# jgrss/cultionet

Hardware: AMD Instinct MI355X
Metric: train_chips_per_sec (higher is better)
Workload: dtype f32

## Files before the change

cultionet_amd/csrc/cn_conv.hip:

```cpp
#include "cn_common.h"
#include "cn_conv_geom.h"
#include "cn_profile.h"

#include <cstdlib>

#define KC 8

static int cn_reduce_slices(const CnConvGeom& g, hipStream_t stream);

template <int TN, int TM>
__device__ __forceinline__ void cn_igemm_epilogue(const CnConvGeom& g, const f32x16 (&acc)[TN][TM],
                                                  const bool (&pix_ok)[TM], const int (&out_off)[TM], int co_base,
                                                  int half, int grp, int split, int b,
                                                  const float* __restrict__ bias, float* __restrict__ y) {
  const int HWout = g.Hout * g.Wout;
  const bool sliced = g.slice_stride != 0;
  float* yb = sliced ? g.part + (long)(grp * g.splits + split) * g.slice_stride + (long)b * g.Cout * HWout
                     : y + (long)b * g.ybs;
  const bool first = split == 0;
#pragma unroll
  for (int tn = 0; tn < TN; ++tn) {
#pragma unroll
    for (int r = 0; r < 16; ++r) {
      const int co = co_base + tn * 32 + (r & 3) + 8 * (r >> 2) + 4 * half;
      if (co < g.Cout) {
        const float bv = (bias != nullptr && first) ? bias[co] : 0.f;
#pragma unroll
        for (int tm = 0; tm < TM; ++tm) {
          if (pix_ok[tm]) {
            float* dst = yb + (long)co * HWout + out_off[tm];
            const float v = acc[tn][tm][r] + bv;
            if (sliced) {
              *dst = acc[tn][tm][r];
            } else if (g.atomic_out) {
              atomicAdd(dst, v);
            } else if (g.accumulate) {
              *dst += v;
            } else {
              *dst = v;
            }
          }
        }
      }
    }
  }
}

template <int WAVES_N, int TN, int NI_T>
__global__ __launch_bounds__(256) void cn_conv_igemm_kernel(const CnConvGeom g) {
  constexpr int WAVES_M = 4 / WAVES_N;
  constexpr int MT = WAVES_M * 64;
  constexpr int NT = WAVES_N * TN * 32;
  constexpr int WI = (CN_MAX_TAPS * KC * (NT / 4) + 255) / 256;
  extern __shared__ __attribute__((aligned(16))) float smem[];
  float* in_lds = smem;
  float* w_lds = smem + g.w_lds_off;
  int* tap_lds = reinterpret_cast<int*>(smem + g.tap_lds_off);

  const int tid = threadIdx.x, lane = tid & 63, wid = tid >> 6;
// ... 131 lines not shown
  {                                                                                                        \
    const float* wrow = w_lds + ((t_) * KC + half) * NT + wn * (TN * 32) + l31;                            \
    _Pragma("unroll") for (int tn = 0; tn < TN; ++tn) opa[bf_][tn] = wrow[(2 * (cp_)) * NT + tn * 32];     \
    opb[bf_][0] = in_lds[pix_lds[0] + (2 * (cp_)) * plane + (toff_)];                                      \
    opb[bf_][1] = in_lds[pix_lds[1] + (2 * (cp_)) * plane + (toff_)];                                      \
  }
#define CN_MFMA(bf_)                                                                                       \
  _Pragma("unroll") for (int tn = 0; tn < TN; ++tn) _Pragma("unroll") for (int tm = 0; tm < 2; ++tm)       \
      acc[tn][tm] = __builtin_amdgcn_mfma_f32_32x32x2f32(opa[bf_][tn], opb[bf_][tm], acc[tn][tm], 0, 0, 0);
      int toff_cur = tap_lds[0];
      CN_LOAD_OPS(0, 0, 0, toff_cur);
#pragma unroll 1
      for (int t = 0; t < ntaps; ++t) {
        const int toff_nxt = (t + 1 < ntaps) ? tap_lds[t + 1] : 0;
        CN_LOAD_OPS(1, t, 1, toff_cur);
        CN_MFMA(0);
        CN_LOAD_OPS(0, t, 2, toff_cur);
        CN_MFMA(1);
        CN_LOAD_OPS(1, t, 3, toff_cur);
        CN_MFMA(0);
        if (t + 1 < ntaps) CN_LOAD_OPS(0, t + 1, 0, toff_nxt);
        CN_MFMA(1);
        toff_cur = toff_nxt;
      }
#undef CN_LOAD_OPS
#undef CN_MFMA
    }
#undef CN_PREFETCH
  }

  cn_igemm_epilogue<TN, 2>(g, acc, pix_ok, out_off, n0 + wn * (TN * 32), half, grp, split, b, bias, y);
}

template <int WAVES_N, int TN, int TM, int NV, int RP>
__global__ __launch_bounds__(256, (NV <= 1 ? 2 : 1)) void cn_conv_igemm_vec_kernel(const CnConvGeom g) {
  constexpr int WAVES_M = 4 / WAVES_N;
  constexpr int MT = WAVES_M * TM * 32;
  constexpr int NT = WAVES_N * TN * 32;
  constexpr int WI = (CN_MAX_TAPS * KC * (NT / 4) + 255) / 256;
  constexpr int VS = NV * 1024;
  constexpr bool PADR = RP == 1 || RP == 2;
  constexpr int ODD = RP == 3 ? 1 : 0;
  constexpr int VSS = VS + ODD;
  extern __shared__ __attribute__((aligned(16))) float smem[];
  float* in_lds = smem;
  float* w_lds = smem + g.w_lds_off;
  int* tap_lds = reinterpret_cast<int*>(smem + g.tap_lds_off);

  const int tid = threadIdx.x, lane = tid & 63, wid = tid >> 6;
  const int half = lane >> 5, l31 = lane & 31;
  const int wm = wid / WAVES_N, wn = wid % WAVES_N;

  int bx, by, split;
  if (!cn_xcd_block(g.grid_x, g.grid_y, g.grid_x * g.grid_y * g.splits, bx, by, split)) return;
  int ci_ = 0;
  if (g.interleave) {
    ci_ = bx % g.ncls;
  } else {
#pragma unroll 1
    for (int c = 1; c < g.ncls; ++c)
      if (bx >= g.cls[c].block_begin) ci_ = c;
  }
  const int grp = g.cls[ci_].grp;
  const float* __restrict__ x = g.gx[grp];
  const float* __restrict__ wp = g.gwp[grp];
  const float* __restrict__ bias = g.gbias[grp];
  float* __restrict__ y = g.gy[grp];
  const int Hg = g.cls[ci_].Hg, Wg = g.cls[ci_].Wg, ntaps = g.cls[ci_].ntaps;
  const int vplane = g.cls[ci_].vplane;
  const int min_dy = g.cls[ci_].min_dy, min_dx = g.cls[ci_].min_dx;
  const int oy0 = g.cls[ci_].oy0, ox0 = g.cls[ci_].ox0;
  const int tiles_per_img = g.cls[ci_].tiles_per_img;
  const int tile = g.interleave ? bx / g.ncls : bx - g.cls[ci_].block_begin;
  const int b = tile / tiles_per_img;
  const int m0 = (tile - b * tiles_per_img) * MT;
  const int Win = g.Win;
  const int pitch = PADR ? ((Win + 3) / 4 * 4 + 4) : Win;
  if (tid < ntaps) {
    tap_lds[tid] = PADR ? (g.cls[ci_].dy[tid] - min_dy) * pitch + g.cls[ci_].dx[tid]
                      : (g.cls[ci_].dy[tid] - min_dy) * Win + (g.cls[ci_].dx[tid] - min_dx);
    tap_lds[CN_MAX_TAPS + tid] = g.cls[ci_].wt[tid];
    tap_lds[2 * CN_MAX_TAPS + tid] = g.cls[ci_].dx[tid];
  }
  __syncthreads();
  const int n0 = by * NT;
  const int Mimg = Hg * Wg;
  const int gy0 = m0 / Wg;
  const int HWin = g.Hin * Win;
  const int start = PADR ? (gy0 * g.is + min_dy) * Win : (gy0 * g.is + min_dy) * Win + min_dx;
  const int f0 = (start >> 2) << 2;
  const int sh = start - f0;

  int goff[NV];
  int ldst[NV];
  int ldst2[NV];
#pragma unroll
  for (int i = 0; i < NV; ++i) {
    const int e4 = 4 * (tid + i * 256) - (PADR ? sh : 0);
    const int lim = PADR ? g.cls[ci_].rows * Win : vplane;
    ldst[i] = 0;
    ldst2[i] = 0;
    if (e4 + 3 >= 0 && e4 < lim) {
      const int fq = start + e4 - (PADR ? 0 : sh);
      goff[i] = (fq >= 0 && (ODD ? fq < HWin : fq + 3 < HWin)) ? fq : -1;
      if (RP == 1) {
        const int r = e4 / Win;
        ldst[i] = r * pitch + 4 + (e4 - r * Win);
      } else if (RP == 2) {
        const int ea = e4 < 0 ? e4 + 2 : e4, eb = e4 + 2;
        const int ra = ea / Win, rb = eb / Win;
        ldst[i] = e4 < 0 ? -1 : ra * pitch + 4 + (ea - ra * Win);
        ldst2[i] = eb < lim ? rb * pitch + 4 + (eb - rb * Win) : -1;
      } else {
        ldst[i] = e4;
      }
    } else {
      goff[i] = -2;
    }
  }
  if (PADR) {
    for (int e = tid; e < KC * VS; e += 256) in_lds[e] = 0.f;
  }

  int pix_lds[TM], out_off[TM];
  unsigned colmask[TM];
  bool pix_ok[TM];
#pragma unroll
  for (int tm = 0; tm < TM; ++tm) {
    const int p = m0 + wm * (TM * 32) + tm * 32 + l31;
    pix_ok[tm] = p < Mimg;
    const int pc = pix_ok[tm] ? p : Mimg - 1;
    const int gy = pc / Wg, gx = pc - gy * Wg;
    pix_lds[tm] = PADR ? ((gy - gy0) * g.is) * pitch + 4 + gx * g.is + half * VS
                     : ((gy - gy0) * g.is) * Win + gx * g.is + sh + half * VSS;
    out_off[tm] = (gy * g.os + oy0) * g.Wout + gx * g.os + ox0;
    unsigned m = 0;
    for (int t = 0; t < ntaps; ++t) {
      const int ix = gx * g.is + tap_lds[2 * CN_MAX_TAPS + t];
      if (ix >= 0 && ix < Win) m |= 1u << t;
    }
    colmask[tm] = m;
  }

  f32x16 acc[TN][TM];
#pragma unroll
  for (int tn = 0; tn < TN; ++tn)
#pragma unroll
    for (int tm = 0; tm < TM; ++tm)
#pragma unroll
      for (int r = 0; r < 16; ++r) acc[tn][tm][r] = 0.f;
  const float* xb = x + (long)b * g.xbs;
  const int nw4 = ntaps * KC * (NT / 4);
  const int nchunks = (g.Cin + KC - 1) / KC;
  int ch = split * g.chunks_per_split;
  int ch_end = ch + g.chunks_per_split;
  if (ch_end > nchunks) ch_end = nchunks;

  if (ntaps > 0 && ch < ch_end) {
    f32x4 xin[KC][NV];
    f32x4 win[WI];
    constexpr unsigned CN_OOB = 0x80000000u;
    const __amdgpu_buffer_rsrc_t xrs =
        __builtin_amdgcn_make_buffer_rsrc(const_cast<float*>(xb), 0, 0x7fffffff, 0x00020000);
    const __amdgpu_buffer_rsrc_t wrs =
        __builtin_amdgcn_make_buffer_rsrc(const_cast<float*>(wp), 0, 0x7fffffff, 0x00020000);
    unsigned xo[NV], wo[WI];
#pragma unroll
    for (int i = 0; i < NV; ++i) xo[i] = goff[i] >= 0 ? (unsigned)goff[i] * 4u : CN_OOB;
#pragma unroll
    for (int j = 0; j < WI; ++j) {
      const int f = tid + j * 256;
      wo[j] = CN_OOB;
      if (f < nw4) {
        const int row = f / (NT / 4), c4 = f - row * (NT / 4);
        const int t = row / KC, ci = row - t * KC;
        wo[j] = (unsigned)(((tap_lds[CN_MAX_TAPS + t] * g.Kpad + ci) * g.Npad + n0 + c4 * 4) * 4);
      }
    }
#define CN_PREFETCH_V(c0_)                                                                                 \
  {                                                                                                        \
    const int c0 = (c0_);                                                                                  \
    _Pragma("unroll") for (int ci = 0; ci < KC; ++ci) {                                                    \
      if ((c0 + ci) < g.Cin) {                                                           \
        const int so = ODD ? (((c0 + ci) * HWin) & ~3) * 4 : (c0 + ci) * HWin * 4;                                                               \
        _Pragma("unroll") for (int i = 0; i < NV; ++i)                                                     \
            xin[ci][i] = __builtin_bit_cast(f32x4, __builtin_amdgcn_raw_buffer_load_b128(xrs, xo[i], so, 0)); \
      } else {                                                                                             \
        _Pragma("unroll") for (int i = 0; i < NV; ++i) xin[ci][i] = f32x4{0.f, 0.f, 0.f, 0.f};             \
      }                                                                                                    \
    }                                                                                                      \
    const int wso = c0 * g.Npad * 4;                                                                       \
    _Pragma("unroll") for (int j = 0; j < WI; ++j)                                                         \
        win[j] = __builtin_bit_cast(f32x4, __builtin_amdgcn_raw_buffer_load_b128(wrs, wo[j], wso, 0));     \
  }
    CN_PREFETCH_V(ch * KC);
    for (; ch < ch_end; ++ch) {
      __syncthreads();
#pragma unroll
      for (int ci = 0; ci < KC; ++ci)
#pragma unroll
        for (int i = 0; i < NV; ++i)
          if (goff[i] != -2) {
            if (RP == 2) {
              if (ldst[i] >= 0) *reinterpret_cast<float2*>(in_lds + ci * VS + ldst[i]) = make_float2(xin[ci][i][0], xin[ci][i][1]);
// ... 17 lines not shown
        if (f < nw4) *reinterpret_cast<f32x4*>(w_lds + f * 4) = win[j];
      }
      __syncthreads();
      if (ch + 1 < ch_end) CN_PREFETCH_V((ch + 1) * KC);
#pragma unroll 1
      for (int t = 0; t < ntaps; ++t) {
        const int toff = tap_lds[t];
        const float* wrow = w_lds + (t * KC + half) * NT + wn * (TN * 32) + l31;
        const float* brow[TM];
        int msk[TM];
#pragma unroll
        for (int tm = 0; tm < TM; ++tm) {
          brow[tm] = in_lds + pix_lds[tm] + toff;
          msk[tm] = PADR ? -1 : __builtin_amdgcn_sbfe((int)colmask[tm], t, 1);
        }
#pragma unroll
        for (int cp = 0; cp < KC / 2; ++cp) {
          float a[TN], bb[TM];
#pragma unroll
          for (int tn = 0; tn < TN; ++tn) a[tn] = wrow[(2 * cp) * NT + tn * 32];
#pragma unroll
          for (int tm = 0; tm < TM; ++tm)
            bb[tm] = PADR ? brow[tm][(2 * cp) * VS] : __int_as_float(__float_as_int(brow[tm][(2 * cp) * VSS]) & msk[tm]);
#pragma unroll
          for (int tn = 0; tn < TN; ++tn)
#pragma unroll
            for (int tm = 0; tm < TM; ++tm)
              acc[tn][tm] = __builtin_amdgcn_mfma_f32_32x32x2f32(a[tn], bb[tm], acc[tn][tm], 0, 0, 0);
        }
      }
    }
#undef CN_PREFETCH_V
  }

  cn_igemm_epilogue<TN, TM>(g, acc, pix_ok, out_off, n0 + wn * (TN * 32), half, grp, split, b, bias, y);
}

__global__ void cn_pack_weights_kernel(const float* __restrict__ w, float* __restrict__ wp, int T, int K,
                                       int N, int Kpad, int Npad, long sk, long sn, long st) {
  const long total = (long)T * Kpad * Npad;
  for (long i = blockIdx.x * (long)blockDim.x + threadIdx.x; i < total; i += (long)gridDim.x * blockDim.x) {
    const int n = (int)(i % Npad);
    const long r = i / Npad;
    const int k = (int)(r % Kpad);
    const int t = (int)(r / Kpad);
    wp[i] = (k < K && n < N) ? w[k * sk + n * sn + t * st] : 0.f;
  }
}

struct CnPackDesc {
  const float* w;
  float* wp;
  int T, K, N, Kpad, Npad;
  long sk, sn, st;
};

#define CN_PK_TS 32
#define CN_PK_PITCH (32 * CN_MAX_TAPS + 1)
__global__ __launch_bounds__(256) void cn_pack_weights_batched_kernel(const CnPackDesc* __restrict__ descs) {
  __shared__ float tile[CN_PK_TS * CN_PK_PITCH];
  const CnPackDesc d = descs[blockIdx.y];
  const bool n_slow = d.sn > d.sk;
  const long ss = n_slow ? d.sn : d.sk, sm = n_slow ? d.sk : d.sn;
  const int S = n_slow ? d.N : d.K, M = n_slow ? d.K : d.N;
  const int Spad = n_slow ? d.Npad : d.Kpad, Mpad = n_slow ? d.Kpad : d.Npad;
  if (d.T > CN_MAX_TAPS || d.st != 1 || sm != d.T) {
    const long total = (long)d.T * d.Kpad * d.Npad;
    for (long i = blockIdx.x * (long)blockDim.x + threadIdx.x; i < total; i += (long)gridDim.x * blockDim.x) {
// ... 33 lines not shown

extern "C" int cn_conv_npad(int n_out) {
  const int nt = cn_pick_nt(n_out);
  return (n_out + nt - 1) / nt * nt;
}
extern "C" int cn_conv_kpad(int k_in) { return (k_in + KC - 1) / KC * KC; }

extern "C" int cn_pack_weights_f32(const float* w, float* wp, int T, int K, int N, long sk, long sn, long st,
                                   void* stream) {
  const int Kpad = cn_conv_kpad(K), Npad = cn_conv_npad(N);
  const long total = (long)T * Kpad * Npad;
  const int blocks = (int)((total + 255) / 256 < 2048 ? (total + 255) / 256 : 2048);
  CN_LAUNCH(cn_pack_weights_kernel, dim3(blocks), dim3(256), 0, (hipStream_t)stream, w, wp, T, K, N,
                     Kpad, Npad, sk, sn, st);
  return cn_check_launch();
}

extern "C" int cn_pack_weights_batched_f32(const void* descs, int n, void* stream) {
  if (n <= 0) return CN_OK;
  CN_LAUNCH(cn_pack_weights_batched_kernel, dim3(64, n), dim3(256), 0, (hipStream_t)stream,
                     (const CnPackDesc*)descs);
  return cn_check_launch();
}

template <int WAVES_N, int TN, int TM, int NV, int RP>
static int cn_launch_igemm_v(const float* x, const float* wp, const float* bias, float* y, CnConvGeom& g,
                             int total_tiles, int max_taps, int splits, double flops, hipStream_t stream) {
  constexpr int NT = WAVES_N * TN * 32;
  g.tap_lds_off = g.w_lds_off + (max_taps > 0 ? max_taps : 1) * KC * NT;
  if ((long)g.Cin * g.Hin * g.Win * 4 >= (1L << 31) || (long)(max_taps > 0 ? max_taps : 1) * g.Kpad * g.Npad * 4 >= (1L << 31))
    return CN_ERR_ARG;
  const size_t lds = (size_t)(g.tap_lds_off + 3 * CN_MAX_TAPS + 1) * sizeof(float);
  if (lds > 160 * 1024) return CN_ERR_LDS;
  static bool attr_set = false;
  if (!attr_set) {
    (void)hipFuncSetAttribute((const void*)cn_conv_igemm_vec_kernel<WAVES_N, TN, TM, NV, RP>,
                              hipFuncAttributeMaxDynamicSharedMemorySize, 160 * 1024);
    attr_set = true;
  }
  g.grid_x = total_tiles;
  g.grid_y = (g.Cout + NT - 1) / NT;
  g.splits = splits < 1 ? 1 : splits;
  dim3 grid(cn_xcd_grid((long)g.grid_x * g.grid_y * g.splits));
  cn_prof_name("cn_conv_igemm_vec_kernel<%d, %d, %d, %d, %d>", WAVES_N, TN, TM, NV, RP);
  cn_prof_desc("igemm_vec<%d,%d,%d,%d,%d> G%d B%d %d->%d %dx%d->%dx%d taps%d cls%d is%d os%d grid%dx%dx%d", WAVES_N, TN,
               TM, NV, RP, g.G, g.B, g.Cin, g.Cout, g.Hin, g.Win, g.Hout, g.Wout, max_taps, g.ncls, g.is, g.os,
               total_tiles, (g.Cout + NT - 1) / NT, splits);
  cn_prof_bytes(4.0 * g.G * ((double)g.B * g.Cin * g.Hin * g.Win + (double)g.B * g.Cout * g.Hout * g.Wout / (g.shared_y ? g.G : 1) +
                             (double)(max_taps > 0 ? max_taps : 1) * g.Cin * g.Cout));
  cn_prof_before(stream);
  CN_LAUNCH((cn_conv_igemm_vec_kernel<WAVES_N, TN, TM, NV, RP>), grid, dim3(256), lds, stream, g);
  cn_prof_after(stream, NT == 128 ? 0 : 1, flops);
  const int rrc = cn_reduce_slices(g, stream);
  return rrc != CN_OK ? rrc : cn_check_launch();
}

template <int WAVES_N, int TN, int NI_T>
static int cn_launch_igemm_t(const float* x, const float* wp, const float* bias, float* y, CnConvGeom& g,
                             int total_tiles, int max_taps, int splits, double flops, hipStream_t stream) {
  constexpr int NT = WAVES_N * TN * 32;
  g.tap_lds_off = g.w_lds_off + (max_taps > 0 ? max_taps : 1) * KC * NT;
  if ((long)g.Cin * g.Hin * g.Win * 4 >= (1L << 31) || (long)(max_taps > 0 ? max_taps : 1) * g.Kpad * g.Npad * 4 >= (1L << 31))
    return CN_ERR_ARG;
  const size_t lds = (size_t)(g.tap_lds_off + 3 * CN_MAX_TAPS + 1) * sizeof(float);
  if (lds > 160 * 1024) return CN_ERR_LDS;
  static bool attr_set = false;
  if (!attr_set) {
    (void)hipFuncSetAttribute((const void*)cn_conv_igemm_kernel<WAVES_N, TN, NI_T>,
                              hipFuncAttributeMaxDynamicSharedMemorySize, 160 * 1024);
    attr_set = true;
  }
  g.grid_x = total_tiles;
  g.grid_y = (g.Cout + NT - 1) / NT;
  g.splits = splits < 1 ? 1 : splits;
  dim3 grid(cn_xcd_grid((long)g.grid_x * g.grid_y * g.splits));
  cn_prof_name("cn_conv_igemm_kernel<%d, %d, %d>", WAVES_N, TN, NI_T);
  cn_prof_desc("igemm_dw<%d,%d,%d> G%d B%d %d->%d %dx%d->%dx%d taps%d cls%d is%d os%d grid%dx%dx%d", WAVES_N, TN, NI_T,
               g.G, g.B, g.Cin, g.Cout, g.Hin, g.Win, g.Hout, g.Wout, max_taps, g.ncls, g.is, g.os, total_tiles,
               (g.Cout + NT - 1) / NT, splits);
  cn_prof_bytes(4.0 * g.G * ((double)g.B * g.Cin * g.Hin * g.Win + (double)g.B * g.Cout * g.Hout * g.Wout / (g.shared_y ? g.G : 1) +
                             (double)(max_taps > 0 ? max_taps : 1) * g.Cin * g.Cout));
  cn_prof_before(stream);
  CN_LAUNCH((cn_conv_igemm_kernel<WAVES_N, TN, NI_T>), grid, dim3(256), lds, stream, g);
  cn_prof_after(stream, NT == 128 ? 0 : 1, flops);
// ... 4 lines not shown
struct CnPlan {
  int total_tiles, max_plane, max_vplane, max_taps;
  int max_rplane, max_absdx;
  double flops;
};

static CnPlan cn_plan(CnConvGeom& g, int MT) {
  CnPlan p = {0, 0, 0, 0, 0, 0, 0.0};
  for (int c = 0; c < g.ncls; ++c) {
    CnConvClass& k = g.cls[c];
    const int Mimg = k.Hg * k.Wg;
    int rows_g = (MT + k.Wg - 2) / k.Wg + 1;
    if (rows_g > k.Hg) rows_g = k.Hg;
    k.min_dy = 0; k.min_dx = 0;
    int max_dy = 0, max_dx = 0;
    for (int t = 0; t < k.ntaps; ++t) {
      if (t == 0 || k.dy[t] < k.min_dy) k.min_dy = k.dy[t];
      if (t == 0 || k.dx[t] < k.min_dx) k.min_dx = k.dx[t];
      if (t == 0 || k.dy[t] > max_dy) max_dy = k.dy[t];
      if (t == 0 || k.dx[t] > max_dx) max_dx = k.dx[t];
    }
    const int rows = (rows_g - 1) * g.is + (max_dy - k.min_dy) + 1;
    k.pitch = (k.Wg - 1) * g.is + (max_dx - k.min_dx) + 1;
    k.plane = rows * k.pitch;
    k.vplane = (rows * g.Win + (max_dx - k.min_dx) + 4 + 3) / 4 * 4;
    k.rows = rows;
    {
      const int rpitch = (g.Win + 3) / 4 * 4 + 4;
      if ((rows + 1) * rpitch + 4 > p.max_rplane) p.max_rplane = (rows + 1) * rpitch + 4;
    }
    if (-k.min_dx > p.max_absdx) p.max_absdx = -k.min_dx;
    if (max_dx > p.max_absdx) p.max_absdx = max_dx;
    k.tiles_per_img = (Mimg + MT - 1) / MT;
    k.block_begin = p.total_tiles;
    p.total_tiles += g.B * k.tiles_per_img;
    if (k.plane > p.max_plane) p.max_plane = k.plane;
    if (k.vplane > p.max_vplane) p.max_vplane = k.vplane;
    if (k.ntaps > p.max_taps) p.max_taps = k.ntaps;
    p.flops += 2.0 * g.B * Mimg * (double)g.Cout * g.Cin * k.ntaps;
  }
  g.interleave = 0;
  if (g.ncls > 1 && g.want_interleave) {
    bool same = true;
    for (int c = 1; c < g.ncls; ++c) same = same && g.cls[c].tiles_per_img == g.cls[0].tiles_per_img;
    g.interleave = same ? 1 : 0;
  }
  return p;
}

struct CnChoice { int cfg, splits, cps; double cost; };

static double cn_launch_cost(long blocks, int cps, double mt_units, int splits, double out_elems) {
  const double F = 273.0, R = 170.0;
  const double c1 = 36.7 + 0.614 * mt_units, c2 = 30.0 + 1.19 * mt_units;
  const long full = blocks / 512, rem = blocks % 512;
  double c = full * (F + cps * c2);
  if (rem > 0) c += F + cps * (rem > 256 ? c2 : c1);
  if (splits > 1) c += R + out_elems * 4.0 * (2.0 * splits + 1.0) / 8.0e6 * (128.0 / 7.5);
  return c;
}

static thread_local float* g_conv_ws;
static thread_local long g_conv_ws_floats;

static CnChoice cn_choose(const CnConvGeom& g0, const int* mts, int ncfg, int NT, bool allow_split) {
  const int nchunks = (g0.Cin + KC - 1) / KC;
  const int ny = (g0.Cout + NT - 1) / NT;
  const int G = g0.G > 0 ? g0.G : 1;
  const double out_elems = (double)g0.B * g0.Cout * g0.Hout * g0.Wout * (g0.shared_y ? 1 : G);
  CnChoice best = {0, 1, nchunks > 0 ? nchunks : 1, 1e300};
  int forced = 0;
  {
    static const char* dbg = getenv("CN_DBG_SPLITS");
    if (dbg) forced = atoi(dbg) < 1 ? 1 : atoi(dbg);
  }
  long ws_cap = 32;
  if (g_conv_ws != nullptr) {
    const long stride = ((long)g0.B * g0.Cout * g0.Hout * g0.Wout + 3) / 4 * 4;
    ws_cap = g_conv_ws_floats / (stride * G);
  }
  int forced_cfg = -1;
  {
    static const char* dbgc = getenv("CN_DBG_CFG");
    if (dbgc) forced_cfg = atoi(dbgc);
  }
  for (int i = 0; i < ncfg; ++i) {
    if (forced_cfg >= 0 && i != (forced_cfg < ncfg ? forced_cfg : ncfg - 1)) continue;
    CnConvGeom gi = g0;
    const CnPlan p = cn_plan(gi, mts[i]);
    if (p.total_tiles <= 0) continue;
    const long base = (long)p.total_tiles * ny;
    int max_splits = (allow_split && p.max_taps > 0 && nchunks >= 4) ? nchunks / 2 : 1;
    if (max_splits > 32) max_splits = 32;
    if (max_splits > ws_cap) max_splits = ws_cap < 1 ? 1 : (int)ws_cap;
    const double taps = p.total_tiles > 0 ? p.flops / (2.0 * g0.Cout * g0.Cin * (double)mts[i] * p.total_tiles) : 9.0;
    const double chunk_units = (double)mts[i] * NT / 128.0 * (taps < 9.0 ? taps : 9.0) / 9.0;
    for (int sp = 1; sp <= max_splits; ++sp) {
      if (forced && sp != (forced > max_splits ? max_splits : forced)) continue;
      const int cps = (nchunks + sp - 1) / sp;
      const int splits = (nchunks + cps - 1) / cps;
      if (splits != sp && !forced) continue;
      const double cost = cn_launch_cost(base * splits, cps, chunk_units, splits, out_elems);
      if (cost < best.cost * (i == best.cfg ? 1.0 : 0.98)) best = {i, splits, cps, cost};
    }
  }
  return best;
}


#include <mutex>
#include <unordered_map>
namespace {
struct CnWs { float* p; long n; };
std::mutex g_ws_mu;
std::unordered_map<void*, CnWs> g_ws_by_stream;
}

extern "C" int cn_conv_set_workspace(void* stream, float* ws, long ws_floats) {
  if (ws != nullptr && ((reinterpret_cast<uintptr_t>(ws) & 15) || ws_floats < 0)) return CN_ERR_ARG;
  std::lock_guard<std::mutex> lk(g_ws_mu);
  if (ws == nullptr) g_ws_by_stream.erase(stream);
  else g_ws_by_stream[stream] = {ws, ws_floats};
  return CN_OK;
}

static void cn_bind_ws(void* stream) {
  std::lock_guard<std::mutex> lk(g_ws_mu);
  auto it = g_ws_by_stream.find(stream);
  if (it == g_ws_by_stream.end()) { g_conv_ws = nullptr; g_conv_ws_floats = 0; }
  else { g_conv_ws = it->second.p; g_conv_ws_floats = it->second.n; }
}

struct CnReduceArgs {
  const float* part;
  long slice_stride;
  int nsum;
  int ngrp;
  float* y[CN_MAX_GROUPS];
  const float* bias[CN_MAX_GROUPS * CN_MAX_GROUPS];
// ... 8 lines not shown
  const float* p0 = a.part + (long)gi * a.nsum * a.slice_stride + (long)b * n;
  float* yb = a.y[gi] + (long)b * a.ybs;
  for (long i = (blockIdx.x * 256L + threadIdx.x) * 4; i < n; i += (long)gridDim.x * 1024) {
    if (i + 3 < n && (n & 3) == 0 && (a.ybs & 3) == 0 && (reinterpret_cast<uintptr_t>(yb) & 15) == 0) {
      f32x4 s = *reinterpret_cast<const f32x4*>(p0 + i);
      for (int k = 1; k < a.nsum; ++k) s += *reinterpret_cast<const f32x4*>(p0 + (long)k * a.slice_stride + i);
#pragma unroll
      for (int e = 0; e < 4; ++e) {
        const int c = (int)((i + e) / a.HW);
        for (int j = 0; j < a.nbias; ++j)
          if (a.bias[gi * CN_MAX_GROUPS + j] != nullptr) s[e] += a.bias[gi * CN_MAX_GROUPS + j][c];
      }
      f32x4* d = reinterpret_cast<f32x4*>(yb + i);
      *d = a.accumulate ? *d + s : s;
    } else {
      for (long e = i; e < n && e < i + 4; ++e) {
        float s = p0[e];
        for (int k = 1; k < a.nsum; ++k) s += p0[(long)k * a.slice_stride + e];
        const int c = (int)(e / a.HW);
        for (int j = 0; j < a.nbias; ++j)
          if (a.bias[gi * CN_MAX_GROUPS + j] != nullptr) s += a.bias[gi * CN_MAX_GROUPS + j][c];
        yb[e] = a.accumulate ? yb[e] + s : s;
      }
    }
  }
}

static int cn_finish_split(CnConvGeom& g, const CnPlan& p, int splits, int cps, float* y, hipStream_t stream) {
  (void)y;
  const int nchunks = (g.Cin + KC - 1) / KC;
  g.chunks_per_split = cps > 0 ? cps : (nchunks > 0 ? nchunks : 1);
  if (p.max_taps == 0) g.chunks_per_split = nchunks > 0 ? nchunks : 1;
  g.splits = splits < 1 ? 1 : splits;
  g.atomic_out = g.splits > 1 || (g.G > 1 && g.shared_y);
  g.part = nullptr;
  g.slice_stride = 0;
  if (g.atomic_out) {
    const long stride = ((long)g.B * g.Cout * g.Hout * g.Wout + 3) / 4 * 4;
    if (g_conv_ws != nullptr && stride * g.G * g.splits <= g_conv_ws_floats) {
      g.part = g_conv_ws;
      g.slice_stride = stride;
      return CN_OK;
    }
  }
  if (g.atomic_out && !g.accumulate) {
    const int ny = g.shared_y ? 1 : g.G;
    for (int i = 0; i < ny; ++i)
      if (hipMemsetAsync(g.gy[i], 0, sizeof(float) * (size_t)g.B * g.Cout * g.Hout * g.Wout, stream) != hipSuccess)
        return CN_ERR_LAUNCH;
  }
  return CN_OK;
}

static int cn_reduce_slices(const CnConvGeom& g, hipStream_t stream) {
  if (g.slice_stride == 0) return CN_OK;
  CnReduceArgs a = {};
  a.part = g.part;
  a.slice_stride = g.slice_stride;
  a.ybs = g.ybs; a.B = g.B; a.Cout = g.Cout; a.HW = g.Hout * g.Wout; a.accumulate = g.accumulate;
  if (g.shared_y) {
    a.nsum = g.G * g.splits; a.ngrp = 1; a.y[0] = g.gy[0]; a.nbias = g.G;
    for (int j = 0; j < g.G; ++j) a.bias[j] = g.gbias[j];
  } else {
    a.nsum = g.splits; a.ngrp = g.G; a.nbias = 1;
    for (int i = 0; i < g.G; ++i) { a.y[i] = g.gy[i]; a.bias[i * CN_MAX_GROUPS] = g.gbias[i]; }
  }
  const long n = (long)g.Cout * a.HW;
  long bx = (n + 1023) / 1024;
  if (bx > 1024) bx = 1024;
  CN_LAUNCH(cn_conv_reduce_kernel, dim3((unsigned)bx, g.B, a.ngrp), dim3(256), 0, stream, a);
  return cn_check_launch();
}

template <int WAVES_N, int TN, int TM>
static int cn_launch_vec_cfg(const float* x, const float* wp, const float* bias, float* y, CnConvGeom& g, int splits,
                             int cps, hipStream_t stream) {
  constexpr int MT = (4 / WAVES_N) * TM * 32;
  const CnPlan p = cn_plan(g, MT);
  if (p.total_tiles <= 0) return CN_OK;
  const int rp = g.odd_planes ? 3
                 : (p.max_rplane <= 4096 && p.max_absdx <= 4) ? (g.Win % 4 == 0 ? 1 : (g.Win % 2 == 0 ? 2 : 0)) : 0;
  const int img = (rp == 1 || rp == 2) ? p.max_rplane : p.max_vplane;
  g.w_lds_off = KC * 1024 * (img <= 1024 ? 1 : (img <= 2048 ? 2 : 4)) + (rp == 3 ? 16 : 0);
  const int rc = cn_finish_split(g, p, splits, cps, y, stream);
  if (rc != CN_OK) return rc;
#define CN_GO(NV_, RP_) \
  return cn_launch_igemm_v<WAVES_N, TN, TM, NV_, RP_>(x, wp, bias, y, g, p.total_tiles, p.max_taps, splits, p.flops, stream)
  if (rp == 1) {
    if (img <= 1024) CN_GO(1, 1);
    if (img <= 2048) CN_GO(2, 1);
    CN_GO(4, 1);
  }
  if (rp == 2) {
    if (img <= 1024) CN_GO(1, 2);
// ... 213 lines not shown
  (void)hipEventDestroy(e0);
  (void)hipEventDestroy(e1);
  return best;
}

int cn_conv_igemm_launch(CnConvGeom& g, hipStream_t stream) {
  if (g.ncls < 1 || g.ncls > CN_MAX_CLASSES || g.B <= 0 || g.G < 1) return g.B <= 0 ? CN_OK : CN_ERR_ARG;
  g.splits = 1;
  const float* x = g.gx[0]; const float* wp = g.gwp[0]; const float* bias = g.gbias[0]; float* y = g.gy[0];
  g.Kpad = cn_conv_kpad(g.Cin);
  g.Npad = cn_conv_npad(g.Cout);
  const int nt = cn_pick_nt(g.Cout);
  const bool dense_out = g.ybs == (long)g.Cout * g.Hout * g.Wout;
  const bool ws_fits = g_conv_ws != nullptr &&
                       (((long)g.B * g.Cout * g.Hout * g.Wout + 3) / 4 * 4) * g.G * 32 <= g_conv_ws_floats;
  const bool allow_split = dense_out || g.accumulate || ws_fits;
  if (g.G > 1 && g.shared_y && !allow_split) return CN_ERR_ARG;
  const int hw4 = (int)(((long)g.Hin * g.Win) % 4);
  g.odd_planes = (hw4 == 1 && !(g.is > 1 && (long)g.Hin * g.Win > 4096)) ? 1 : 0;
  bool vec = (hw4 == 0 || g.odd_planes) && (g.xbs % 4 == 0);
  if (g.is > 1 && (long)g.Hin * g.Win > 4096) vec = false;
  if ((long)g.Cin * g.Hin * g.Win * 4 >= (1L << 31) || (long)CN_MAX_TAPS * cn_conv_kpad(g.Cin) * g.Npad * 4 >= (1L << 31))
    return CN_ERR_ARG;
  for (int i = 0; i < g.G; ++i) vec = vec && ((reinterpret_cast<uintptr_t>(g.gx[i]) & 15) == 0);
  if (vec) {
    CnConvGeom t = g;
    vec = cn_plan(t, 256).max_vplane <= 4 * 1024;
  }
  static const int mts128[3] = {128, 96, 160};
  static const int mts128d[1] = {128};
  static const int mts256[1] = {256};
  const int* mts = nt == 128 ? (vec ? mts128 : mts128d) : mts256;
  const int ncfg = (nt == 128 && vec) ? 3 : 1;
  auto run = [&](const CnChoice& c, CnConvGeom& gg) -> int {
    if (nt == 128) {
      if (vec) {
        switch (c.cfg) {
          case 1: return cn_launch_vec_cfg<4, 1, 3>(x, wp, bias, y, gg, c.splits, c.cps, stream);
          case 2: return cn_launch_vec_cfg<4, 1, 5>(x, wp, bias, y, gg, c.splits, c.cps, stream);
          default: return cn_launch_vec_cfg<2, 2, 2>(x, wp, bias, y, gg, c.splits, c.cps, stream);
        }
      }
      return cn_launch_dword_cfg<2, 2>(x, wp, bias, y, gg, c.splits, c.cps, stream);
    }
    int rc;
    if (nt == 64) {
      if (vec) return cn_launch_vec_cfg<1, 2, 2>(x, wp, bias, y, gg, c.splits, c.cps, stream);
      rc = cn_launch_dword_cfg<1, 2>(x, wp, bias, y, gg, c.splits, c.cps, stream);
    } else {
      if (vec) return cn_launch_vec_cfg<1, 1, 2>(x, wp, bias, y, gg, c.splits, c.cps, stream);
      rc = cn_launch_dword_cfg<1, 1>(x, wp, bias, y, gg, c.splits, c.cps, stream);
    }
    if (rc == CN_ERR_LDS) {
      CnConvGeom g2 = gg;
      rc = cn_launch_dword_cfg<2, 2>(x, wp, bias, y, g2, c.splits, c.cps, stream);
    }
    return rc;
  };
  CnChoice c = cn_choose(g, mts, ncfg, nt, allow_split);
  if (g_autotune) {
    std::lock_guard<std::mutex> lk(g_tune_mu);
    const uint64_t key = cn_tune_key(g, vec, nt, allow_split);
    auto it = g_tuned.find(key);
    if (it != g_tuned.end()) {
      c = it->second;
    } else if (!g.accumulate && !cn_prof_on()) {
      c = cn_autotune(g, mts, ncfg, nt, allow_split, c, run, stream);
      g_tuned.emplace(key, c);
    }
  }
  return run(c, g);
}

static int cn_set_groups(CnConvGeom& g, int G, const float* const* xs, const float* const* wps,
                         const float* const* biases, float* const* ys) {
  if (G < 1 || G > CN_MAX_GROUPS) return CN_ERR_ARG;
  g.G = G;
  int same = 0;
  for (int i = 0; i < G; ++i) {
    g.gx[i] = xs[i]; g.gwp[i] = wps[i]; g.gbias[i] = biases ? biases[i] : nullptr; g.gy[i] = ys[i];
    if (ys[i] == ys[0]) ++same;
  }
  if (same != G && same != 1) return CN_ERR_ARG;
  for (int i = 1; i < G && same == 1; ++i)
    for (int j = 1; j < i; ++j)
      if (ys[i] == ys[j]) return CN_ERR_ARG;
  g.shared_y = (G > 1 && same == G) ? 1 : 0;
  g.has_bias = 0;
  for (int i = 0; i < G; ++i) g.has_bias |= g.gbias[i] != nullptr;
  return CN_OK;
}

// ... 214 lines not shown
```

cultionet_amd/csrc/cn_conv_geom.h:

```cpp
#pragma once
#define CN_MAX_TAPS 9
#define CN_MAX_CLASSES 16
#define CN_MAX_GROUPS 4

struct CnConvClass {
  int Hg, Wg;
  int oy0, ox0;
  int ntaps;
  int dy[CN_MAX_TAPS], dx[CN_MAX_TAPS], wt[CN_MAX_TAPS];
  int min_dy, min_dx;
  int pitch, plane;
  int vplane;
  int rows;
  int tiles_per_img;
  int block_begin;
  int grp;
};

struct CnConvGeom {
  int B, Cin, Hin, Win;
  int Cout, Hout, Wout;
  long xbs, ybs;
  int is, os;
  int Kpad, Npad;
  int w_lds_off;
  int tap_lds_off;
  int chunks_per_split;
  int atomic_out;
  int accumulate, has_bias;
  int G, splits, shared_y;
  int odd_planes;
  int want_interleave;
  int interleave;
  float* part;
  long slice_stride;
  int grid_x, grid_y;
  const float* gx[CN_MAX_GROUPS];
  const float* gwp[CN_MAX_GROUPS];
  const float* gbias[CN_MAX_GROUPS];
  float* gy[CN_MAX_GROUPS];
  int ncls;
  CnConvClass cls[CN_MAX_CLASSES];
};

static inline int cn_conv_out(int in, int k, int stride, int pad, int dil) {
  return (in + 2 * pad - dil * (k - 1) - 1) / stride + 1;
}
static inline int cn_convt_out(int in, int k, int stride, int pad, int out_pad) {
  return (in - 1) * stride - 2 * pad + k + out_pad;
}
static inline int cn_floordiv(int a, int b) { return (a >= 0) ? a / b : -((-a + b - 1) / b); }

static inline int cn_gather_taps(int KH, int KW, int pad, int dil, int* dy, int* dx, int* wt) {
  for (int ky = 0; ky < KH; ++ky)
    for (int kx = 0; kx < KW; ++kx) {
      const int t = ky * KW + kx;
      dy[t] = ky * dil - pad; dx[t] = kx * dil - pad; wt[t] = t;
    }
  return KH * KW;
}

static inline int cn_parity_extent(int out, int p, int stride) { return (out - p + stride - 1) / stride; }

static inline int cn_parity_taps(int py, int px, int KH, int KW, int stride, int pad, int dil, int* dy, int* dx,
                                 int* wt) {
  int nt = 0;
// ... 23 lines not shown
```

Baseline: 382.2.

## Fold grouped shared-output convolutions into one K-loop per tile

Adds a FOLD variant of the vectorized implicit-GEMM conv kernel. When several groups write into the same output and share geometry, one block iterates over every group's input channels and accumulates in registers instead of each group atomically adding or writing a separate slice. All group biases are summed in the epilogue. The cost model picks fold or no fold per shape. This removes atomics and slice reductions but gives fewer, longer blocks and an extra per-group tap-table setup with syncs.

After: 383.2, median of 4. No clear change (+0.3%).

```diff
diff --git a/cultionet_amd/csrc/cn_conv.hip b/cultionet_amd/csrc/cn_conv.hip
--- a/cultionet_amd/csrc/cn_conv.hip
+++ b/cultionet_amd/csrc/cn_conv.hip
@@ -8,7 +8,7 @@
 
 static int cn_reduce_slices(const CnConvGeom& g, hipStream_t stream);
 
-template <int TN, int TM>
+template <int TN, int TM, bool FOLD = false>
 __device__ __forceinline__ void cn_igemm_epilogue(const CnConvGeom& g, const f32x16 (&acc)[TN][TM],
                                                   const bool (&pix_ok)[TM], const int (&out_off)[TM], int co_base,
                                                   int half, int grp, int split, int b,
@@ -24,7 +24,12 @@
     for (int r = 0; r < 16; ++r) {
       const int co = co_base + tn * 32 + (r & 3) + 8 * (r >> 2) + 4 * half;
       if (co < g.Cout) {
-        const float bv = (bias != nullptr && first) ? bias[co] : 0.f;
+        float bv = (bias != nullptr && first) ? bias[co] : 0.f;
+        if (FOLD && first) {
+#pragma unroll
+          for (int j = 1; j < CN_MAX_GROUPS; ++j)
+            if (j < g.G && g.gbias[j] != nullptr) bv += g.gbias[j][co];
+        }
 #pragma unroll
         for (int tm = 0; tm < TM; ++tm) {
           if (pix_ok[tm]) {
@@ -222,7 +227,7 @@
   cn_igemm_epilogue<TN, 2>(g, acc, pix_ok, out_off, n0 + wn * (TN * 32), half, grp, split, b, bias, y);
 }
 
-template <int WAVES_N, int TN, int TM, int NV, int RP>
+template <int WAVES_N, int TN, int TM, int NV, int RP, bool FOLD>
 __global__ __launch_bounds__(256, (NV <= 1 ? 2 : 1)) void cn_conv_igemm_vec_kernel(const CnConvGeom g) {
   constexpr int WAVES_M = 4 / WAVES_N;
   constexpr int MT = WAVES_M * TM * 32;
@@ -244,39 +249,73 @@
   int bx, by, split;
   if (!cn_xcd_block(g.grid_x, g.grid_y, g.grid_x * g.grid_y * g.splits, bx, by, split)) return;
   int ci_ = 0;
-  if (g.interleave) {
+  if (FOLD) {
+  } else if (g.interleave) {
     ci_ = bx % g.ncls;
   } else {
 #pragma unroll 1
     for (int c = 1; c < g.ncls; ++c)
       if (bx >= g.cls[c].block_begin) ci_ = c;
   }
-  const int grp = g.cls[ci_].grp;
-  const float* __restrict__ x = g.gx[grp];
-  const float* __restrict__ wp = g.gwp[grp];
-  const float* __restrict__ bias = g.gbias[grp];
-  float* __restrict__ y = g.gy[grp];
-  const int Hg = g.cls[ci_].Hg, Wg = g.cls[ci_].Wg, ntaps = g.cls[ci_].ntaps;
-  const int vplane = g.cls[ci_].vplane;
-  const int min_dy = g.cls[ci_].min_dy, min_dx = g.cls[ci_].min_dx;
+  const int Hg = g.cls[ci_].Hg, Wg = g.cls[ci_].Wg;
   const int oy0 = g.cls[ci_].oy0, ox0 = g.cls[ci_].ox0;
   const int tiles_per_img = g.cls[ci_].tiles_per_img;
-  const int tile = g.interleave ? bx / g.ncls : bx - g.cls[ci_].block_begin;
+  const int tile = FOLD ? bx : (g.interleave ? bx / g.ncls : bx - g.cls[ci_].block_begin);
   const int b = tile / tiles_per_img;
   const int m0 = (tile - b * tiles_per_img) * MT;
   const int Win = g.Win;
   const int pitch = PADR ? ((Win + 3) / 4 * 4 + 4) : Win;
-  if (tid < ntaps) {
-    tap_lds[tid] = PADR ? (g.cls[ci_].dy[tid] - min_dy) * pitch + g.cls[ci_].dx[tid]
-                      : (g.cls[ci_].dy[tid] - min_dy) * Win + (g.cls[ci_].dx[tid] - min_dx);
-    tap_lds[CN_MAX_TAPS + tid] = g.cls[ci_].wt[tid];
-    tap_lds[2 * CN_MAX_TAPS + tid] = g.cls[ci_].dx[tid];
-  }
-  __syncthreads();
   const int n0 = by * NT;
   const int Mimg = Hg * Wg;
   const int gy0 = m0 / Wg;
   const int HWin = g.Hin * Win;
+
+  int out_off[TM];
+  bool pix_ok[TM];
+#define CN_OUT_TILE()                                                  \
+  _Pragma("unroll") for (int tm = 0; tm < TM; ++tm) {                  \
+    const int p = m0 + wm * (TM * 32) + tm * 32 + l31;                 \
+    pix_ok[tm] = p < Mimg;                                             \
+    const int pc = pix_ok[tm] ? p : Mimg - 1;                          \
+    const int gy = pc / Wg, gx = pc - gy * Wg;                         \
+    out_off[tm] = (gy * g.os + oy0) * g.Wout + gx * g.os + ox0;        \
+  }
+  if (!FOLD) CN_OUT_TILE();
+
+  f32x16 acc[TN][TM];
+#pragma unroll
+  for (int tn = 0; tn < TN; ++tn)
+#pragma unroll
+    for (int tm = 0; tm < TM; ++tm)
+#pragma unroll
+      for (int r = 0; r < 16; ++r) acc[tn][tm][r] = 0.f;
+
+  const int nchunks = (g.Cin + KC - 1) / KC;
+  const int c_lo = split * g.chunks_per_split;
+  int c_hi = c_lo + g.chunks_per_split;
+  if (c_hi > (FOLD ? g.ncls : 1) * nchunks) c_hi = (FOLD ? g.ncls : 1) * nchunks;
+  const int k_first = FOLD ? c_lo / nchunks : ci_;
+  const int k_last = FOLD ? (c_hi - 1) / nchunks : ci_;
+
+#pragma unroll 1
+  for (int kc = k_first; kc <= k_last; ++kc) {
+  const int grp = g.cls[kc].grp;
+  const float* __restrict__ x = g.gx[grp];
+  const float* __restrict__ wp = g.gwp[grp];
+  const int ntaps = g.cls[kc].ntaps;
+  const int vplane = g.cls[kc].vplane;
+  const int min_dy = g.cls[kc].min_dy, min_dx = g.cls[kc].min_dx;
+  int tk = tid;
+  if (FOLD) asm volatile("" : "+v"(tk));
+  const int kl31 = tk & 31, khalf = (tk & 63) >> 5, kwm = (tk >> 6) / WAVES_N;
+  if (FOLD) __syncthreads();
+  if (tid < ntaps) {
+    tap_lds[tid] = PADR ? (g.cls[kc].dy[tid] - min_dy) * pitch + g.cls[kc].dx[tid]
+                      : (g.cls[kc].dy[tid] - min_dy) * Win + (g.cls[kc].dx[tid] - min_dx);
+    tap_lds[CN_MAX_TAPS + tid] = g.cls[kc].wt[tid];
+    tap_lds[2 * CN_MAX_TAPS + tid] = g.cls[kc].dx[tid];
+  }
+  __syncthreads();
   const int start = PADR ? (gy0 * g.is + min_dy) * Win : (gy0 * g.is + min_dy) * Win + min_dx;
   const int f0 = (start >> 2) << 2;
   const int sh = start - f0;
@@ -286,8 +325,8 @@
   int ldst2[NV];
 #pragma unroll
   for (int i = 0; i < NV; ++i) {
-    const int e4 = 4 * (tid + i * 256) - (PADR ? sh : 0);
-    const int lim = PADR ? g.cls[ci_].rows * Win : vplane;
+    const int e4 = 4 * (tk + i * 256) - (PADR ? sh : 0);
+    const int lim = PADR ? g.cls[kc].rows * Win : vplane;
     ldst[i] = 0;
     ldst2[i] = 0;
     if (e4 + 3 >= 0 && e4 < lim) {
@@ -308,22 +347,19 @@
       goff[i] = -2;
     }
   }
-  if (PADR) {
+  if (PADR && (!FOLD || kc == k_first)) {
     for (int e = tid; e < KC * VS; e += 256) in_lds[e] = 0.f;
   }
 
-  int pix_lds[TM], out_off[TM];
+  int pix_lds[TM];
   unsigned colmask[TM];
-  bool pix_ok[TM];
 #pragma unroll
   for (int tm = 0; tm < TM; ++tm) {
-    const int p = m0 + wm * (TM * 32) + tm * 32 + l31;
-    pix_ok[tm] = p < Mimg;
-    const int pc = pix_ok[tm] ? p : Mimg - 1;
+    const int p = m0 + kwm * (TM * 32) + tm * 32 + kl31;
+    const int pc = p < Mimg ? p : Mimg - 1;
     const int gy = pc / Wg, gx = pc - gy * Wg;
-    pix_lds[tm] = PADR ? ((gy - gy0) * g.is) * pitch + 4 + gx * g.is + half * VS
-                     : ((gy - gy0) * g.is) * Win + gx * g.is + sh + half * VSS;
-    out_off[tm] = (gy * g.os + oy0) * g.Wout + gx * g.os + ox0;
+    pix_lds[tm] = PADR ? ((gy - gy0) * g.is) * pitch + 4 + gx * g.is + khalf * VS
+                     : ((gy - gy0) * g.is) * Win + gx * g.is + sh + khalf * VSS;
     unsigned m = 0;
     for (int t = 0; t < ntaps; ++t) {
       const int ix = gx * g.is + tap_lds[2 * CN_MAX_TAPS + t];
@@ -332,18 +368,11 @@
     colmask[tm] = m;
   }
 
-  f32x16 acc[TN][TM];
-#pragma unroll
-  for (int tn = 0; tn < TN; ++tn)
-#pragma unroll
-    for (int tm = 0; tm < TM; ++tm)
-#pragma unroll
-      for (int r = 0; r < 16; ++r) acc[tn][tm][r] = 0.f;
   const float* xb = x + (long)b * g.xbs;
   const int nw4 = ntaps * KC * (NT / 4);
-  const int nchunks = (g.Cin + KC - 1) / KC;
-  int ch = split * g.chunks_per_split;
-  int ch_end = ch + g.chunks_per_split;
+  int ch = FOLD ? c_lo - kc * nchunks : c_lo;
+  int ch_end = FOLD ? c_hi - kc * nchunks : c_hi;
+  if (ch < 0) ch = 0;
   if (ch_end > nchunks) ch_end = nchunks;
 
   if (ntaps > 0 && ch < ch_end) {
@@ -359,7 +388,7 @@
     for (int i = 0; i < NV; ++i) xo[i] = goff[i] >= 0 ? (unsigned)goff[i] * 4u : CN_OOB;
 #pragma unroll
     for (int j = 0; j < WI; ++j) {
-      const int f = tid + j * 256;
+      const int f = tk + j * 256;
       wo[j] = CN_OOB;
       if (f < nw4) {
         const int row = f / (NT / 4), c4 = f - row * (NT / 4);
@@ -443,8 +472,13 @@
     }
 #undef CN_PREFETCH_V
   }
-
-  cn_igemm_epilogue<TN, TM>(g, acc, pix_ok, out_off, n0 + wn * (TN * 32), half, grp, split, b, bias, y);
+  }
+  if (FOLD) CN_OUT_TILE();
+#undef CN_OUT_TILE
+
+  const int ogrp = FOLD ? 0 : g.cls[ci_].grp;
+  cn_igemm_epilogue<TN, TM, FOLD>(g, acc, pix_ok, out_off, n0 + wn * (TN * 32), half, ogrp, split, b, g.gbias[ogrp],
+                            g.gy[ogrp]);
 }
 
 __global__ void cn_pack_weights_kernel(const float* __restrict__ w, float* __restrict__ wp, int T, int K,
@@ -544,24 +578,31 @@
     return CN_ERR_ARG;
   const size_t lds = (size_t)(g.tap_lds_off + 3 * CN_MAX_TAPS + 1) * sizeof(float);
   if (lds > 160 * 1024) return CN_ERR_LDS;
-  static bool attr_set = false;
-  if (!attr_set) {
-    (void)hipFuncSetAttribute((const void*)cn_conv_igemm_vec_kernel<WAVES_N, TN, TM, NV, RP>,
-                              hipFuncAttributeMaxDynamicSharedMemorySize, 160 * 1024);
-    attr_set = true;
+  static bool attr_set[2] = {false, false};
+  if (!attr_set[g.fold ? 1 : 0]) {
+    if (g.fold)
+      (void)hipFuncSetAttribute((const void*)cn_conv_igemm_vec_kernel<WAVES_N, TN, TM, NV, RP, true>,
+                                hipFuncAttributeMaxDynamicSharedMemorySize, 160 * 1024);
+    else
+      (void)hipFuncSetAttribute((const void*)cn_conv_igemm_vec_kernel<WAVES_N, TN, TM, NV, RP, false>,
+                                hipFuncAttributeMaxDynamicSharedMemorySize, 160 * 1024);
+    attr_set[g.fold ? 1 : 0] = true;
   }
   g.grid_x = total_tiles;
   g.grid_y = (g.Cout + NT - 1) / NT;
   g.splits = splits < 1 ? 1 : splits;
   dim3 grid(cn_xcd_grid((long)g.grid_x * g.grid_y * g.splits));
   cn_prof_name("cn_conv_igemm_vec_kernel<%d, %d, %d, %d, %d>", WAVES_N, TN, TM, NV, RP);
-  cn_prof_desc("igemm_vec<%d,%d,%d,%d,%d> G%d B%d %d->%d %dx%d->%dx%d taps%d cls%d is%d os%d grid%dx%dx%d", WAVES_N, TN,
+  cn_prof_desc("igemm_vec<%d,%d,%d,%d,%d> G%d B%d %d->%d %dx%d->%dx%d taps%d cls%d is%d os%d grid%dx%dx%d%s", WAVES_N, TN,
                TM, NV, RP, g.G, g.B, g.Cin, g.Cout, g.Hin, g.Win, g.Hout, g.Wout, max_taps, g.ncls, g.is, g.os,
-               total_tiles, (g.Cout + NT - 1) / NT, splits);
+               total_tiles, (g.Cout + NT - 1) / NT, splits, g.fold ? " fold" : "");
   cn_prof_bytes(4.0 * g.G * ((double)g.B * g.Cin * g.Hin * g.Win + (double)g.B * g.Cout * g.Hout * g.Wout / (g.shared_y ? g.G : 1) +
                              (double)(max_taps > 0 ? max_taps : 1) * g.Cin * g.Cout));
   cn_prof_before(stream);
-  CN_LAUNCH((cn_conv_igemm_vec_kernel<WAVES_N, TN, TM, NV, RP>), grid, dim3(256), lds, stream, g);
+  if (g.fold)
+    CN_LAUNCH((cn_conv_igemm_vec_kernel<WAVES_N, TN, TM, NV, RP, true>), grid, dim3(256), lds, stream, g);
+  else
+    CN_LAUNCH((cn_conv_igemm_vec_kernel<WAVES_N, TN, TM, NV, RP, false>), grid, dim3(256), lds, stream, g);
   cn_prof_after(stream, NT == 128 ? 0 : 1, flops);
   const int rrc = cn_reduce_slices(g, stream);
   return rrc != CN_OK ? rrc : cn_check_launch();
@@ -632,8 +673,8 @@
     if (-k.min_dx > p.max_absdx) p.max_absdx = -k.min_dx;
     if (max_dx > p.max_absdx) p.max_absdx = max_dx;
     k.tiles_per_img = (Mimg + MT - 1) / MT;
-    k.block_begin = p.total_tiles;
-    p.total_tiles += g.B * k.tiles_per_img;
+    k.block_begin = g.fold ? 0 : p.total_tiles;
+    if (!g.fold || c == 0) p.total_tiles += g.B * k.tiles_per_img;
     if (k.plane > p.max_plane) p.max_plane = k.plane;
     if (k.vplane > p.max_vplane) p.max_vplane = k.vplane;
     if (k.ntaps > p.max_taps) p.max_taps = k.ntaps;
@@ -648,7 +689,19 @@
   return p;
 }
 
-struct CnChoice { int cfg, splits, cps; double cost; };
+struct CnChoice { int cfg, splits, cps; double cost; int fold; long cfg_blocks; };
+
+static bool cn_fold_legal(const CnConvGeom& g) {
+  if (g.G < 2 || !g.shared_y || g.os != 1 || g.ncls != g.G || g.Cin <= 0 || g.want_interleave) return false;
+  unsigned seen = 0;
+  for (int c = 0; c < g.ncls; ++c) {
+    const CnConvClass& k = g.cls[c];
+    if (k.Hg != g.cls[0].Hg || k.Wg != g.cls[0].Wg || k.oy0 != g.cls[0].oy0 || k.ox0 != g.cls[0].ox0) return false;
+    if (k.grp < 0 || k.grp >= g.G) return false;
+    seen |= 1u << k.grp;
+  }
+  return seen == (1u << g.G) - 1u;
+}
 
 static double cn_launch_cost(long blocks, int cps, double mt_units, int splits, double out_elems) {
   const double F = 273.0, R = 170.0;
@@ -663,48 +716,69 @@
 static thread_local float* g_conv_ws;
 static thread_local long g_conv_ws_floats;
 
-static CnChoice cn_choose(const CnConvGeom& g0, const int* mts, int ncfg, int NT, bool allow_split) {
+static CnChoice cn_choose(const CnConvGeom& g0, const int* mts, int ncfg, int NT, bool allow_split, bool may_fold) {
   const int nchunks = (g0.Cin + KC - 1) / KC;
   const int ny = (g0.Cout + NT - 1) / NT;
   const int G = g0.G > 0 ? g0.G : 1;
   const double out_elems = (double)g0.B * g0.Cout * g0.Hout * g0.Wout * (g0.shared_y ? 1 : G);
-  CnChoice best = {0, 1, nchunks > 0 ? nchunks : 1, 1e300};
   int forced = 0;
   {
     static const char* dbg = getenv("CN_DBG_SPLITS");
     if (dbg) forced = atoi(dbg) < 1 ? 1 : atoi(dbg);
   }
-  long ws_cap = 32;
-  if (g_conv_ws != nullptr) {
-    const long stride = ((long)g0.B * g0.Cout * g0.Hout * g0.Wout + 3) / 4 * 4;
-    ws_cap = g_conv_ws_floats / (stride * G);
-  }
   int forced_cfg = -1;
   {
     static const char* dbgc = getenv("CN_DBG_CFG");
     if (dbgc) forced_cfg = atoi(dbgc);
   }
-  for (int i = 0; i < ncfg; ++i) {
-    if (forced_cfg >= 0 && i != (forced_cfg < ncfg ? forced_cfg : ncfg - 1)) continue;
-    CnConvGeom gi = g0;
-    const CnPlan p = cn_plan(gi, mts[i]);
-    if (p.total_tiles <= 0) continue;
-    const long base = (long)p.total_tiles * ny;
-    int max_splits = (allow_split && p.max_taps > 0 && nchunks >= 4) ? nchunks / 2 : 1;
-    if (max_splits > 32) max_splits = 32;
-    if (max_splits > ws_cap) max_splits = ws_cap < 1 ? 1 : (int)ws_cap;
-    const double taps = p.total_tiles > 0 ? p.flops / (2.0 * g0.Cout * g0.Cin * (double)mts[i] * p.total_tiles) : 9.0;
-    const double chunk_units = (double)mts[i] * NT / 128.0 * (taps < 9.0 ? taps : 9.0) / 9.0;
-    for (int sp = 1; sp <= max_splits; ++sp) {
-      if (forced && sp != (forced > max_splits ? max_splits : forced)) continue;
-      const int cps = (nchunks + sp - 1) / sp;
-      const int splits = (nchunks + cps - 1) / cps;
-      if (splits != sp && !forced) continue;
-      const double cost = cn_launch_cost(base * splits, cps, chunk_units, splits, out_elems);
-      if (cost < best.cost * (i == best.cfg ? 1.0 : 0.98)) best = {i, splits, cps, cost};
-    }
-  }
-  return best;
+  int forced_fold = -1;
+  {
+    static const char* dbgf = getenv("CN_DBG_FOLD");
+    if (dbgf) forced_fold = atoi(dbgf) != 0 ? 1 : 0;
+  }
+  if (forced_fold == 0) may_fold = false;
+  CnChoice bests[2] = {{0, 1, nchunks > 0 ? nchunks : 1, 1e300, 0, 0}, {0, 1, G * (nchunks > 0 ? nchunks : 1), 1e300, 1, 0}};
+  for (int fo = 0; fo < (may_fold ? 2 : 1); ++fo) {
+    CnChoice& best = bests[fo];
+    const int nch = fo ? G * nchunks : nchunks;
+    long ws_cap = 32;
+    if (g_conv_ws != nullptr) {
+      const long stride = ((long)g0.B * g0.Cout * g0.Hout * g0.Wout + 3) / 4 * 4;
+      ws_cap = g_conv_ws_floats / (stride * (fo ? 1 : G));
+    }
+    for (int i = 0; i < ncfg; ++i) {
+      if (forced_cfg >= 0 && i != (forced_cfg < ncfg ? forced_cfg : ncfg - 1)) continue;
+      CnConvGeom gi = g0;
+      gi.fold = fo;
+      const CnPlan p = cn_plan(gi, mts[i]);
+      if (p.total_tiles <= 0) continue;
+      const long base = (long)p.total_tiles * ny;
+      int max_splits = (allow_split && p.max_taps > 0 && nch >= 4) ? nch / 2 : 1;
+      if (max_splits > 32) max_splits = 32;
+      if (max_splits > ws_cap) max_splits = ws_cap < 1 ? 1 : (int)ws_cap;
+      const double taps = p.flops / (2.0 * g0.Cout * g0.Cin * (double)mts[i] * p.total_tiles * (fo ? G : 1));
+      const double chunk_units = (double)mts[i] * NT / 128.0 * (taps < 9.0 ? taps : 9.0) / 9.0;
+      for (int sp = 1; sp <= max_splits; ++sp) {
+        if (forced && sp != (forced > max_splits ? max_splits : forced)) continue;
+        const int cps = (nch + sp - 1) / sp;
+        const int splits = (nch + cps - 1) / cps;
+        if (splits != sp && !forced) continue;
+        if (fo && forced_fold != 1 && base * splits < (long)bests[0].cfg_blocks) continue;
+        double cost = cn_launch_cost(base * splits, cps, chunk_units, splits, out_elems);
+        if (fo) cost += (double)((base * splits + 511) / 512) * (G - 1) * 40.0;
+        if (cost < best.cost * (i == best.cfg ? 1.0 : 0.98)) best = {i, splits, cps, cost, fo, base * splits};
+      }
+    }
+  }
+  if (!may_fold || bests[1].cost >= 1e300) return bests[0];
+  if (forced_fold == 1 || bests[0].cost >= 1e300) return bests[1];
+  const double R = 170.0;
+  const double slice_units = out_elems * 4.0 / 8.0e6 * (128.0 / 7.5);
+  const int s0 = bests[0].splits;
+  const long stride0 = ((long)g0.B * g0.Cout * g0.Hout * g0.Wout + 3) / 4 * 4;
+  const bool sliced0 = g_conv_ws != nullptr && stride0 * G * s0 <= g_conv_ws_floats;
+  const double behind = !sliced0 ? 0.0 : (s0 > 1 ? 0.0 : R + 3.0 * slice_units) + 2.0 * (G - 1) * s0 * slice_units;
+  return bests[1].cost < 0.98 * (bests[0].cost + behind) ? bests[1] : bests[0];
 }
 
 
@@ -779,12 +853,16 @@
   g.chunks_per_split = cps > 0 ? cps : (nchunks > 0 ? nchunks : 1);
   if (p.max_taps == 0) g.chunks_per_split = nchunks > 0 ? nchunks : 1;
   g.splits = splits < 1 ? 1 : splits;
-  g.atomic_out = g.splits > 1 || (g.G > 1 && g.shared_y);
+  if (g.fold) {
+    const int all = g.G * (nchunks > 0 ? nchunks : 1);
+    if (cps <= 0 || p.max_taps == 0) g.chunks_per_split = all;
+  }
+  g.atomic_out = g.splits > 1 || (g.G > 1 && g.shared_y && !g.fold);
   g.part = nullptr;
   g.slice_stride = 0;
   if (g.atomic_out) {
     const long stride = ((long)g.B * g.Cout * g.Hout * g.Wout + 3) / 4 * 4;
-    if (g_conv_ws != nullptr && stride * g.G * g.splits <= g_conv_ws_floats) {
+    if (g_conv_ws != nullptr && stride * (g.fold ? 1 : g.G) * g.splits <= g_conv_ws_floats) {
       g.part = g_conv_ws;
       g.slice_stride = stride;
       return CN_OK;
@@ -806,7 +884,7 @@
   a.slice_stride = g.slice_stride;
   a.ybs = g.ybs; a.B = g.B; a.Cout = g.Cout; a.HW = g.Hout * g.Wout; a.accumulate = g.accumulate;
   if (g.shared_y) {
-    a.nsum = g.G * g.splits; a.ngrp = 1; a.y[0] = g.gy[0]; a.nbias = g.G;
+    a.nsum = (g.fold ? 1 : g.G) * g.splits; a.ngrp = 1; a.y[0] = g.gy[0]; a.nbias = g.G;
     for (int j = 0; j < g.G; ++j) a.bias[j] = g.gbias[j];
   } else {
     a.nsum = g.splits; a.ngrp = g.G; a.nbias = 1;
@@ -1086,7 +1164,9 @@
   static const int mts256[1] = {256};
   const int* mts = nt == 128 ? (vec ? mts128 : mts128d) : mts256;
   const int ncfg = (nt == 128 && vec) ? 3 : 1;
+  const bool may_fold = vec && cn_fold_legal(g);
   auto run = [&](const CnChoice& c, CnConvGeom& gg) -> int {
+    gg.fold = (may_fold && c.fold) ? 1 : 0;
     if (nt == 128) {
       if (vec) {
         switch (c.cfg) {
@@ -1111,7 +1191,7 @@
     }
     return rc;
   };
-  CnChoice c = cn_choose(g, mts, ncfg, nt, allow_split);
+  CnChoice c = cn_choose(g, mts, ncfg, nt, allow_split, may_fold);
   if (g_autotune) {
     std::lock_guard<std::mutex> lk(g_tune_mu);
     const uint64_t key = cn_tune_key(g, vec, nt, allow_split);
diff --git a/cultionet_amd/csrc/cn_conv_geom.h b/cultionet_amd/csrc/cn_conv_geom.h
--- a/cultionet_amd/csrc/cn_conv_geom.h
+++ b/cultionet_amd/csrc/cn_conv_geom.h
@@ -32,6 +32,7 @@
   int odd_planes;
   int want_interleave;
   int interleave;
+  int fold;
   float* part;
   long slice_stride;
   int grid_x, grid_y;
```
